# DakeQQ/Voice-Activity-Detection-VAD-ONNX

Hardware: AMD Instinct MI355X
Metric: audio frames/sec/GPU (16 kHz, 512-sample hop); RTF at batch=1 (higher is better)
Workload: dtype f32; 1 GPU; Silero-VAD f32, batch=4096 synthetic 10 s @16 kHz clips per GPU (STFT conv + conv1d stack + LSTM cell HIP, seeded synthetic weights); clips_per_gpu=4096, samples_per_clip=160000, frames_per_clip=313, parallelism=clip-sharded x1, no collective

## Files before the change

voice-activity-detection-vad-onnx_amd/csrc/silero.hip:

```cpp
#include "silero_common.h"
#include "split_scheme.h"

#include <math.h>
#include <stddef.h>
#include <stdlib.h>
#include <string.h>

namespace vadx {
namespace silero {

constexpr int ENCODER_DEFAULT = 2;

constexpr int V_LD = 100, A1_LD = 68, A2_LD = 36, A3_LD = 20, A4_LD = 20;
constexpr int V_SCR = 129 * V_LD;
constexpr int R0_FLOATS = V_SCR + 256;
constexpr int A2_OFF = 128 * A1_LD;
constexpr int A3_OFF = 0, A4_OFF = 64 * A3_LD;
constexpr int ENC_LDS_FLOATS = R0_FLOATS;
static_assert(16 * X_LDM <= R0_FLOATS && A2_OFF + 64 * A2_LD <= R0_FLOATS && 3 * ENC_LDS_FLOATS * 4 <= 160 * 1024, "encoder LDS map");

__device__ constexpr float WINO_BT[6][4] = {{0.f, -5.f, 0.f, 1.f}, {-4.f, -4.f, 1.f, 1.f}, {4.f, -4.f, -1.f, 1.f},
                                            {-2.f, -1.f, 2.f, 1.f}, {2.f, -1.f, -2.f, 1.f}, {4.f, 0.f, -5.f, 0.f}};
constexpr int ENC_THREADS = 512;

// ... 362 lines not shown
    }
    __syncthreads();

    {
        const f32x4 a4 = gemm_chain<0, 4, 4, 4>(A3, A3_LD, P + OFF_C4 + wave * 4 * FRAG + lane * 4, lane, [](int) { return 0; });
        const float bias = P[OFF_B4 + wave * 16 + i];
        f32x4 v;
#pragma unroll
        for (int r = 0; r < 4; ++r) v[r] = fmaxf(a4[r] + bias, 0.f);
        *reinterpret_cast<f32x4 *>(&A4[(wave * 16 + i) * A4_LD + 4 * q]) = v;
    }
    __syncthreads();

    {
        f32x4 acc[4][1];
#pragma unroll
        for (int g = 0; g < 4; ++g)
            acc[g][0] = *reinterpret_cast<const f32x4 *>(P + OFF_BG + g * 128 + wave * 16 + 4 * q);
        {
            const float *wl = P + OFF_IH + wave * 8 * FRAG + lane * 4;
            const float *ap = A4 + (4 * q) * A4_LD + i;
            f32x4 wcur[4], wnxt[4];
#pragma unroll
            for (int g = 0; g < 4; ++g) wcur[g] = *reinterpret_cast<const f32x4 *>(wl + g * 64 * FRAG);
#pragma unroll
            for (int S = 0; S < 8; ++S) {
                const int Sn = (S + 1 < 8) ? S + 1 : S;
#pragma unroll
                for (int g = 0; g < 4; ++g) wnxt[g] = *reinterpret_cast<const f32x4 *>(wl + g * 64 * FRAG + Sn * FRAG);
                __builtin_amdgcn_sched_barrier(0);
                const float *aps = ap + 16 * S * A4_LD;
#pragma unroll
                for (int j = 0; j < 4; ++j) {
                    const float av = aps[j * A4_LD];
#pragma unroll
                    for (int g = 0; g < 4; ++g) acc[g][0] = mfma16(wcur[g][j], av, acc[g][0]);
                }
#pragma unroll
                for (int g = 0; g < 4; ++g) wcur[g] = wnxt[g];
            }
        }
        float *dst = gx + ((size_t)t * Gws + g0 + grp) * GX_TILE_FLOATS + (size_t)wave * 4 * 256 + lane * 4;
#pragma unroll
        for (int g = 0; g < 4; ++g)
            *reinterpret_cast<f32x4 *>(dst + g * 256) = acc[g][0];
    }
}

constexpr int HS_LD = 136;
constexpr int LSTM_LDS_FLOATS = 2 * 16 * HS_LD + 2 * 8 * 16;
constexpr int LSTM_THREADS = 512;

__global__ __launch_bounds__(LSTM_THREADS, 2) void silero_lstm_kernel(
    const float *__restrict__ P, const float *__restrict__ gx, const float *__restrict__ state0,
    int B, int G, int T, float *__restrict__ probs, long long probs_stride,
    float *__restrict__ state_n) {
    extern __shared__ __attribute__((aligned(16))) float lds[];
    float *Hs = lds;
    float *part = lds + 2 * 16 * HS_LD;

    const int tid = threadIdx.x, lane = tid & 63, wave = tid >> 6;
    const int q = lane >> 4, n = lane & 15;
    const int grp = blockIdx.x;
    const long long b = (long long)grp * 16 + n;
    const bool bvalid = b < B;
    const int u0 = wave * 16 + 4 * q;

    float a[4][32];
#pragma unroll
    for (int g = 0; g < 4; ++g) {
        const float *row = P + OFF_HH + (g * 128 + wave * 16 + n) * 128 + 4 * q;
#pragma unroll
        for (int S = 0; S < 8; ++S) {
            const f32x4 w4 = *reinterpret_cast<const f32x4 *>(row + 16 * S);
            a[g][4 * S + 0] = w4[0]; a[g][4 * S + 1] = w4[1]; a[g][4 * S + 2] = w4[2]; a[g][4 * S + 3] = w4[3];
        }
    }
    f32x4 dw = *reinterpret_cast<const f32x4 *>(P + OFF_DW + u0);
    const float db = P[OFF_DB];

    f32x4 c = {0.f, 0.f, 0.f, 0.f}, h = {0.f, 0.f, 0.f, 0.f};
    if (state0 != nullptr && bvalid) {
        h = *reinterpret_cast<const f32x4 *>(state0 + b * 128 + u0);
        c = *reinterpret_cast<const f32x4 *>(state0 + ((long long)B + b) * 128 + u0);
    }
    *reinterpret_cast<f32x4 *>(&Hs[n * HS_LD + u0]) = h;
    __syncthreads();

    const float *gsrc = gx + (size_t)grp * GX_TILE_FLOATS + (size_t)wave * 4 * 256 + lane * 4;
    const size_t gstep = (size_t)G * GX_TILE_FLOATS;
    f32x4 gcur[4], gnxt[4];
#pragma unroll
    for (int g = 0; g < 4; ++g) gcur[g] = *reinterpret_cast<const f32x4 *>(gsrc + g * 256);

    int cur = 0;
    for (int t = 0; t < T; ++t) {
        const int tn = (t + 1 < T) ? t + 1 : t;
#pragma unroll
        for (int g = 0; g < 4; ++g) gnxt[g] = *reinterpret_cast<const f32x4 *>(gsrc + tn * gstep + g * 256);

        const float *hb = Hs + cur * 16 * HS_LD + n * HS_LD + 4 * q;
        f32x4 hv[8];
#pragma unroll
        for (int S = 0; S < 8; ++S) hv[S] = *reinterpret_cast<const f32x4 *>(hb + 16 * S);
        auto gate = [&](int g) {
            f32x4 acc = gcur[g];
#pragma unroll
            for (int S = 0; S < 8; ++S)
#pragma unroll
                for (int j = 0; j < 4; ++j) acc = mfma16(a[g][4 * S + j], hv[S][j], acc);
            return acc;
        };
        const f32x4 ai = gate(0), af = gate(1);
        f32x4 ig, fg, gg;
#pragma unroll
        for (int r = 0; r < 4; ++r) ig[r] = gate_sigmoid(ai[r]);
        const f32x4 ag = gate(2);
#pragma unroll
        for (int r = 0; r < 4; ++r) fg[r] = gate_sigmoid(af[r]);
        const f32x4 ao = gate(3);
        float dpart = 0.f;
#pragma unroll
        for (int r = 0; r < 4; ++r) {
            gg[r] = gate_tanh(ag[r]);
            c[r] = fg[r] * c[r] + ig[r] * gg[r];
        }
#pragma unroll
        for (int r = 0; r < 4; ++r) {
            h[r] = gate_sigmoid(ao[r]) * gate_tanh(c[r]);
            dpart = fmaf(dw[r], fmaxf(h[r], 0.f), dpart);
        }
        const int nxt = cur ^ 1;
        *reinterpret_cast<f32x4 *>(&Hs[nxt * 16 * HS_LD + n * HS_LD + u0]) = h;
        dpart += __shfl_xor(dpart, 16);
        dpart += __shfl_xor(dpart, 32);
        if (q == 0) part[(nxt * 8 + wave) * 16 + n] = dpart;
        __syncthreads();
        if (wave == 0 && lane < 16 && bvalid) {
            float s = db;
#pragma unroll
            for (int w = 0; w < 8; ++w) s += part[(nxt * 8 + w) * 16 + lane];
            probs[b * probs_stride + t] = sigmoidf_(s);
        }
        cur = nxt;
#pragma unroll
        for (int g = 0; g < 4; ++g) gcur[g] = gnxt[g];
    }
    if (state_n != nullptr && bvalid) {
        *reinterpret_cast<f32x4 *>(state_n + b * 128 + u0) = h;
        *reinterpret_cast<f32x4 *>(state_n + ((long long)B + b) * 128 + u0) = c;
    }
}

constexpr int SEG_CLIPS = 16;
__global__ void silero_segments_kernel(const float *__restrict__ probs, int B, int T,
                                       const long long *__restrict__ n_samples,
                                       vadx_silero_seg_params prm, long long *__restrict__ segs,
                                       int *__restrict__ counts, int cap) {
    const int b = blockIdx.x * blockDim.x + threadIdx.x;
    if (b >= B) return;
    const double sr = (double)prm.sampling_rate;
    const long long W = (prm.sampling_rate == 16000) ? 512 : 256;
    const double thr = prm.threshold;
    const double neg = (prm.neg_threshold < 0.0) ? fmax(thr - 0.15, 0.01) : prm.neg_threshold;
    const double min_speech = sr * prm.min_speech_duration_ms / 1000.0;
    const double pad = sr * prm.speech_pad_ms / 1000.0;
    const double max_speech = sr * prm.max_speech_duration_s - (double)W - 2.0 * pad;
    const double min_sil = sr * prm.min_silence_duration_ms / 1000.0;
    const double min_sil_at_max = sr * prm.min_silence_at_max_speech / 1000.0;
    const long long L = n_samples[b];
    const int nwin = (int)((L + W - 1) / W) < T ? (int)((L + W - 1) / W) : T;

    long long *out = segs + (size_t)b * cap * 2;
    int ns = 0;
    auto push = [&](long long s, long long e) {
        if (ns < cap) { out[2 * ns] = s; out[2 * ns + 1] = e; }
        ++ns;
    };

    auto win_floor = [&](double x) { const double q = floor(x / (double)W); return q >= 2147483647.0 ? 2147483647 : (q <= -2147483648.0 ? (int)-2147483647 - 1 : (int)q); };
    auto win_ceil = [&](double x) { const double q = ceil(x / (double)W); return q >= 2147483647.0 ? 2147483647 : (q <= -2147483648.0 ? (int)-2147483647 - 1 : (int)q); };
    auto f32_not_below = [](double x) { float f = (float)x; if ((double)f < x) f = nextafterf(f, INFINITY); return f; };
    const float thr_f = f32_not_below(thr), neg_f = f32_not_below(neg);
    const int d_sil_at_max = win_floor(min_sil_at_max), d_max_speech = win_floor(max_speech), d_min_sil = win_ceil(min_sil),
              d_min_speech = win_floor(min_speech);
    auto pushw = [&](int s_, int e_) { push((long long)s_ * W, (long long)e_ * W); };

    bool triggered = false, have_cur = false, have_possible = false;
    int cur_start = 0, temp_end = 0, prev_end = 0, next_start = 0;
    int best_end = 0, best_dur = 0;
    auto step = [&](int pos, float p) {
        if (p >= thr_f && temp_end) {
            const int gap = pos - temp_end;
            if (gap > d_sil_at_max) {
                if (!have_possible || gap > best_dur) { best_end = temp_end; best_dur = gap; }
                have_possible = true;
            }
            temp_end = 0;
            if (next_start < prev_end) next_start = pos;
        }
        if (p >= thr_f && !triggered) {
            triggered = true; cur_start = pos; have_cur = true;
            return;
        }
        if (triggered && (pos - cur_start) > d_max_speech) {
            if (prm.use_max_poss_sil_at_max_speech && have_possible) {
                prev_end = best_end;
                pushw(cur_start, prev_end);
                have_cur = false;
                next_start = prev_end + best_dur;
                if (next_start < prev_end + pos) { cur_start = next_start; have_cur = true; }
                else triggered = false;
                prev_end = next_start = temp_end = 0;
                have_possible = false;
            } else if (prev_end) {
                pushw(cur_start, prev_end);
                have_cur = false;
                if (next_start < prev_end) triggered = false;
                else { cur_start = next_start; have_cur = true; }
                prev_end = next_start = temp_end = 0;
                have_possible = false;
            } else {
                pushw(cur_start, pos);
                have_cur = false;
                prev_end = next_start = temp_end = 0;
                triggered = false;
                have_possible = false;
                return;
            }
        }
        if (p < neg_f && triggered) {
            if (!temp_end) temp_end = pos;
            const int sil_now = pos - temp_end;
            if (!prm.use_max_poss_sil_at_max_speech && sil_now > d_sil_at_max) prev_end = temp_end;
            if (sil_now < d_min_sil) return;
            if ((temp_end - cur_start) > d_min_speech) pushw(cur_start, temp_end);
            have_cur = false;
            prev_end = next_start = temp_end = 0;
            triggered = false;
            have_possible = false;
            return;
        }
        };
    const float *pr = probs + (size_t)b * T;
    for (int k0 = 0; k0 < nwin; k0 += 8) {
        float buf[8];
#pragma unroll
        for (int j = 0; j < 8; ++j) buf[j] = pr[k0 + j < T ? k0 + j : T - 1];
#pragma unroll
        for (int j = 0; j < 8; ++j)
            if (k0 + j < nwin) step(k0 + j, buf[j]);
    }
    if (have_cur && (double)(L - (long long)cur_start * W) > min_speech) push((long long)cur_start * W, L);

    const int m = ns < cap ? ns : cap;
    for (int s = 0; s < m; ++s) {
        if (s == 0) out[0] = (long long)fmax(0.0, (double)out[0] - pad);
        if (s != m - 1) {
            const long long gap = out[2 * (s + 1)] - out[2 * s + 1];
            if ((double)gap < 2.0 * pad) {
                const long long half = gap >= 0 ? gap / 2 : -((-gap + 1) / 2);
                out[2 * s + 1] += half;
                const long long ns0 = out[2 * (s + 1)] - half;
                out[2 * (s + 1)] = ns0 > 0 ? ns0 : 0;
            } else {
                out[2 * s + 1] = (long long)fmin((double)L, (double)out[2 * s + 1] + pad);
                out[2 * (s + 1)] = (long long)fmax(0.0, (double)out[2 * (s + 1)] - pad);
            }
        } else {
            out[2 * s + 1] = (long long)fmin((double)L, (double)out[2 * s + 1] + pad);
        }
    }
    counts[b] = ns;
}


}
}

using namespace vadx::silero;
using vadx::FRAG;

#define VADX_SILERO_ARITH(cfg, who)                                                                               \
    const int arith = vadx::arith_internal((cfg) ? (cfg)->arithmetic : VADX_ARITH_AUTO, ENCODER_DEFAULT);         \
    VADX_REQUIRE(arith >= 0, who ": cfg->arithmetic=%d is not one of VADX_ARITH_*", (cfg) ? (cfg)->arithmetic : 0)
static_assert(sizeof(vadx_silero_cfg) == 16 && offsetof(vadx_silero_cfg, ext) == 4 && sizeof(((vadx_silero_cfg *)nullptr)->ext) == 12,
              "vadx_silero_cfg layout");
static int rate_of(const vadx_silero_cfg *cfg) {
    const int r = cfg ? cfg->ext.sample_rate : 0;
    return (r == 0 || r == 16000) ? 16000 : (r == 8000 ? 8000 : -1);
}
#define VADX_SILERO_RATE(cfg, who)                                                                                \
    const int rate = rate_of(cfg);                                                                                \
    VADX_REQUIRE(rate > 0, who ": cfg->ext.sample_rate=%d is not 16000 or 8000 (0 = 16000)", (cfg) ? (cfg)->ext.sample_rate : 0); \
    const long long win = rate == 8000 ? 256 : 512, ctx = win / 8

extern "C" int vadx_silero_range_flag(const float *packed, int reset, uint32_t *flag_host, float *amax_host, void *stream) {
    VADX_REQUIRE(packed && flag_host, "vadx_silero_range_flag: NULL argument");
    return vadx::range_flag_read(packed + OFF_HFLAG + 1, reset, flag_host, amax_host, stream);
}

extern "C" size_t vadx_silero_workspace_bytes(int batch, int steps) {
    if (batch <= 0 || steps <= 0) return 0;
    const size_t G = ((size_t)batch + 15) / 16;
    return G * (size_t)steps * GX_TILE_FLOATS * sizeof(float);
}

template <typename S>
int vadx::silero::silero_encode_launch(const float *packed, const S *src, float in_scale, long long n_valid, long long row_stride,
                                       long long origin, int batch, int steps, void *ws, size_t ws_bytes, void *stream,
                                       const vadx_silero_cfg *cfg, int first_group, int total_batch) {
    VADX_SILERO_ARITH(cfg, "silero");
    VADX_SILERO_RATE(cfg, "silero");
    (void)ctx;
    VADX_REQUIRE(packed && src && ws, "silero: NULL pointer argument");
    VADX_REQUIRE(batch > 0 && steps > 0, "silero: batch=%d steps=%d must be positive", batch, steps);
    VADX_REQUIRE((reinterpret_cast<uintptr_t>(packed) & 15) == 0 && (reinterpret_cast<uintptr_t>(ws) & 15) == 0,
                 "silero: packed weights and workspace must be 16-byte aligned");
    if (total_batch <= 0) total_batch = batch;
    const int Gws = (total_batch + 15) / 16;
    const int G = (batch + 15) / 16;
    VADX_REQUIRE(first_group >= 0 && first_group + G <= Gws, "silero: clip groups [%d, %d) outside the workspace's %d", first_group,
                 first_group + G, Gws);
    if (ws_bytes < vadx_silero_workspace_bytes(total_batch, steps)) {
        vadx::set_error("silero: workspace %zu B < required %zu B", ws_bytes, vadx_silero_workspace_bytes(total_batch, steps));
        return VADX_ENOSPACE;
    }
    const long long nblk = (long long)G * steps;
    VADX_REQUIRE(nblk < (1LL << 31), "silero: too many tiles (%lld)", nblk);
    if (win == 256)
        return silero8k_encode_launch<S>(arith, packed, src, in_scale, n_valid, row_stride, origin, batch, G, steps, Gws, first_group,
                                         static_cast<float *>(ws), stream);
    if (arith == 2)
        return silero_encode_h2_launch<S>(packed, src, in_scale, n_valid, row_stride, origin, batch, G, steps, Gws, first_group,
                                          static_cast<float *>(ws), stream);
    if (arith == 1)
        return silero_encode_split_launch<S>(packed, src, in_scale, n_valid, row_stride, origin, batch, G, steps, Gws, first_group,
                                             static_cast<float *>(ws), stream);
    VADX_DYN_LDS(silero_encode_kernel<S>, ENC_LDS_FLOATS * sizeof(float));
    hipLaunchKernelGGL(silero_encode_kernel<S>, dim3((unsigned)nblk), dim3(ENC_THREADS), ENC_LDS_FLOATS * sizeof(float),
                       static_cast<hipStream_t>(stream), packed, src, in_scale, n_valid, row_stride, origin, batch, G, steps,
                       Gws, first_group, static_cast<float *>(ws));
    VADX_HIP_TRY(hipGetLastError());
    return VADX_OK;
}

int vadx::silero::silero_recur_launch(const float *packed, const void *ws, size_t ws_bytes, int batch, int steps,
                                      const float *state0, float *probs, long long probs_stride, float *state_n, void *stream,
                                      const vadx_silero_cfg *cfg) {
    VADX_SILERO_ARITH(cfg, "silero");
    VADX_SILERO_RATE(cfg, "silero");
    (void)win; (void)ctx;
    VADX_REQUIRE(packed && ws && probs, "silero: NULL pointer argument");
    VADX_REQUIRE(batch > 0 && steps > 0, "silero: batch=%d steps=%d must be positive", batch, steps);
    if (ws_bytes < vadx_silero_workspace_bytes(batch, steps)) {
        vadx::set_error("silero: workspace %zu B < required %zu B", ws_bytes, vadx_silero_workspace_bytes(batch, steps));
        return VADX_ENOSPACE;
    }
    const int G = (batch + 15) / 16;
    if (arith == 2)
        return silero_lstm_h2_launch(packed, static_cast<const float *>(ws), state0, batch, G, steps, probs, probs_stride, state_n, stream);
    if (arith == 1)
        return silero_lstm_split_launch(packed, static_cast<const float *>(ws), state0, batch, G, steps, probs, probs_stride, state_n, stream);
    hipLaunchKernelGGL(silero_lstm_kernel, dim3(G), dim3(LSTM_THREADS), LSTM_LDS_FLOATS * sizeof(float),
                       static_cast<hipStream_t>(stream), packed, static_cast<const float *>(ws), state0, batch, G, steps,
                       probs, probs_stride, state_n);
    VADX_HIP_TRY(hipGetLastError());
    return VADX_OK;
}

template int vadx::silero::silero_encode_launch<float>(const float *, const float *, float, long long, long long, long long, int, int,
                                                       void *, size_t, void *, const vadx_silero_cfg *, int, int);
template int vadx::silero::silero_encode_launch<int16_t>(const float *, const int16_t *, float, long long, long long, long long, int, int,
                                                         void *, size_t, void *, const vadx_silero_cfg *, int, int);

static int silero_run(const float *packed, const float *src, long long n_valid, long long row_stride,
                      long long origin, int batch, int steps, const float *state0, float *probs,
                      long long probs_stride, float *state_n, void *ws, size_t ws_bytes, void *stream, const vadx_silero_cfg *cfg) {
    int rc = silero_encode_launch(packed, src, 1.0f, n_valid, row_stride, origin, batch, steps, ws, ws_bytes, stream, cfg);
    if (rc != VADX_OK) return rc;
    return silero_recur_launch(packed, ws, ws_bytes, batch, steps, state0, probs, probs_stride, state_n, stream, cfg);
}

extern "C" int vadx_silero_encode(const float *packed, const float *audio, int batch, int64_t n_samples,
                                  int64_t row_stride, void *workspace, size_t workspace_bytes, void *stream, const vadx_silero_cfg *cfg) {
    VADX_SILERO_RATE(cfg, "vadx_silero_encode");
    VADX_REQUIRE(n_samples > 0 && row_stride >= n_samples, "vadx_silero_encode: n_samples=%lld row_stride=%lld",
                 (long long)n_samples, (long long)row_stride);
    const long long steps = (n_samples + win - 1) / win;
    VADX_REQUIRE(steps < (1LL << 30), "vadx_silero_encode: clip too long");
    return silero_encode_launch(packed, audio, 1.0f, n_samples, row_stride, -ctx, batch, (int)steps, workspace, workspace_bytes, stream, cfg);
}

extern "C" int vadx_silero_encode_pcm16(const float *packed, const int16_t *audio, float scale, int batch, int64_t n_samples,
                                        int64_t row_stride, void *workspace, size_t workspace_bytes, void *stream, const vadx_silero_cfg *cfg) {
    VADX_SILERO_RATE(cfg, "vadx_silero_encode_pcm16");
    VADX_REQUIRE(n_samples > 0 && row_stride >= n_samples, "vadx_silero_encode_pcm16: n_samples=%lld row_stride=%lld",
                 (long long)n_samples, (long long)row_stride);
    const long long steps = (n_samples + win - 1) / win;
    VADX_REQUIRE(steps < (1LL << 30), "vadx_silero_encode_pcm16: clip too long");
    return silero_encode_launch(packed, audio, scale, n_samples, row_stride, -ctx, batch, (int)steps, workspace, workspace_bytes, stream, cfg);
}

extern "C" int vadx_silero_encode_pcm16_part(const float *packed, const int16_t *audio, float scale, int batch, int64_t n_samples,
                                             int64_t row_stride, int first_clip, int total_batch, void *workspace,
                                             size_t workspace_bytes, void *stream, const vadx_silero_cfg *cfg) {
    VADX_SILERO_RATE(cfg, "vadx_silero_encode_pcm16_part");
    VADX_REQUIRE(n_samples > 0 && row_stride >= n_samples, "vadx_silero_encode_pcm16_part: n_samples=%lld row_stride=%lld",
                 (long long)n_samples, (long long)row_stride);
    VADX_REQUIRE(first_clip >= 0 && first_clip % 16 == 0 && first_clip + batch <= total_batch,
                 "vadx_silero_encode_pcm16_part: first_clip=%d must be a multiple of 16 and first_clip + batch <= total_batch=%d",
                 first_clip, total_batch);
    const long long steps = (n_samples + win - 1) / win;
    VADX_REQUIRE(steps < (1LL << 30), "vadx_silero_encode_pcm16_part: clip too long");
    return silero_encode_launch(packed, audio, scale, n_samples, row_stride, -ctx, batch, (int)steps, workspace, workspace_bytes, stream,
                                cfg, first_clip / 16, total_batch);
}

extern "C" int vadx_silero_recur(const float *packed, const void *workspace, size_t workspace_bytes, int batch,
                                 int steps, const float *state0, float *probs, float *state_n, void *stream, const vadx_silero_cfg *cfg) {
    return silero_recur_launch(packed, workspace, workspace_bytes, batch, steps, state0, probs, steps, state_n, stream, cfg);
}

extern "C" int vadx_silero_encode_span(const float *packed, const float *audio, int batch, int64_t n_samples,
                                       int64_t row_stride, int first_step, int n_steps, void *workspace,
                                       size_t workspace_bytes, void *stream, const vadx_silero_cfg *cfg) {
    VADX_SILERO_RATE(cfg, "vadx_silero_encode_span");
    VADX_REQUIRE(n_samples > 0 && row_stride >= n_samples, "vadx_silero_encode_span: n_samples=%lld row_stride=%lld",
                 (long long)n_samples, (long long)row_stride);
    const long long steps = (n_samples + win - 1) / win;
    VADX_REQUIRE(first_step >= 0 && n_steps > 0 && (long long)first_step + n_steps <= steps,
                 "vadx_silero_encode_span: span [%d, %d + %d) outside the clip's %lld windows", first_step, first_step, n_steps, steps);
    return silero_encode_launch(packed, audio, 1.0f, n_samples, row_stride, (long long)first_step * win - ctx, batch, n_steps,
                                workspace, workspace_bytes, stream, cfg);
}

extern "C" int vadx_silero_recur_span(const float *packed, const void *workspace, size_t workspace_bytes, int batch,
                                      int n_steps, const float *state0, float *probs, int64_t probs_stride,
                                      float *state_n, void *stream, const vadx_silero_cfg *cfg) {
    VADX_REQUIRE(probs_stride >= n_steps, "vadx_silero_recur_span: probs_stride=%lld < n_steps=%d", (long long)probs_stride, n_steps);
    return silero_recur_launch(packed, workspace, workspace_bytes, batch, n_steps, state0, probs, probs_stride, state_n, stream, cfg);
}

extern "C" int vadx_silero_step(const float *packed, const float *input, const float *state, int64_t sr,
                                int batch, float *out, float *state_n, void *workspace,
                                size_t workspace_bytes, void *stream, const vadx_silero_cfg *cfg) {
    VADX_SILERO_RATE(cfg, "vadx_silero_step");
    VADX_REQUIRE(sr == rate, "Supported sampling rates: [%d] (got %lld; vadx_silero_cfg.ext.sample_rate selects the network)", rate, (long long)sr);
    VADX_REQUIRE(state && state_n, "vadx_silero_step: state / state_n must not be NULL");
    return silero_run(packed, input, win + ctx, win + ctx, 0, batch, 1, state, out, 1, state_n, workspace, workspace_bytes, stream, cfg);
}

extern "C" int vadx_silero_clips(const float *packed, const float *audio, int batch, int64_t n_samples,
                                 int64_t row_stride, float *probs, float *state_n, void *workspace,
                                 size_t workspace_bytes, void *stream, const vadx_silero_cfg *cfg) {
    VADX_SILERO_RATE(cfg, "vadx_silero_clips");
    VADX_REQUIRE(n_samples > 0 && row_stride >= n_samples, "vadx_silero_clips: n_samples=%lld row_stride=%lld",
                 (long long)n_samples, (long long)row_stride);
    const long long steps = (n_samples + win - 1) / win;
    VADX_REQUIRE(steps < (1LL << 30), "vadx_silero_clips: clip too long");
    return silero_run(packed, audio, n_samples, row_stride, -ctx, batch, (int)steps, nullptr, probs, steps,
                      state_n, workspace, workspace_bytes, stream, cfg);
}

extern "C" int vadx_silero_segments(const float *probs, int batch, int steps, const int64_t *n_samples,
                                    const vadx_silero_seg_params *params, int64_t *segments,
                                    int32_t *counts, int cap, void *stream) {
    VADX_REQUIRE(probs && n_samples && params && segments && counts, "vadx_silero_segments: NULL pointer argument");
    VADX_REQUIRE(batch > 0 && steps > 0 && cap > 0, "vadx_silero_segments: batch/steps/cap must be positive");
    VADX_REQUIRE(params->sampling_rate == 16000 || params->sampling_rate == 8000,
                 "Currently silero VAD models support 8000 and 16000 (or multiply of 16000) sample rates");
    hipLaunchKernelGGL(silero_segments_kernel, dim3((batch + SEG_CLIPS - 1) / SEG_CLIPS), dim3(SEG_CLIPS), 0, static_cast<hipStream_t>(stream),
                       probs, batch, steps, reinterpret_cast<const long long *>(n_samples), *params,
                       reinterpret_cast<long long *>(segments), counts, cap);
    VADX_HIP_TRY(hipGetLastError());
    return VADX_OK;
}
```

voice-activity-detection-vad-onnx_amd/csrc/silero_h2.hip:

```cpp
#include "silero_common.h"
#include "split2.h"

#define H2_IDS()                                                                                           \
    int t_ = tid0;                                                                                         \
    asm volatile("" : "+v"(t_));                                                                           \
    const int tid = t_, lane = tid & 63, wave = tid >> 6, q = lane >> 4, i = lane & 15;                    \
    (void)tid; (void)lane; (void)wave; (void)q; (void)i

namespace vadx {
namespace silero {

constexpr int H2_THREADS = 512;
constexpr int H2_WAVES_PER_SIMD = 4;
constexpr int H2_AHS = 2, H2_AH1 = 2;
constexpr int H2_EO_PL = 8192, H2_EO_KG = 1024;
constexpr int H2_PL128 = 16384, H2_FR128 = 4096;
constexpr int H2_SCR = 32768;
constexpr int H2_EXC2 = 36864, H2_EXC3 = 45056;
constexpr int H2_C2 = 53248, H2_PL2 = 4096, H2_FR2 = 2048;
constexpr int H2_R1 = 65536, H2_T3 = 4096, H2_PL3 = 2048;
constexpr int H2_C4 = 0, H2_T4 = 8192, H2_PL4 = 4096;
constexpr int H2_NSUB = 4;
constexpr int H2_LDS_BYTES = H2_R1 + H2_NSUB * H2_T3;
static_assert(16 * X_LDM * 4 <= H2_EXC3 && H2_EXC3 + 4096 <= H2_C2 && H2_C2 + 2 * H2_PL2 <= H2_R1, "fp16 x 2 encoder LDS map: a tile");
// ... 356 lines not shown
            }
        }
        f32x4 s2[2] = {join2(hi[0], mid[0]), join2(hi[1], mid[1])};
        float *exc = reinterpret_cast<float *>(smem + H2_EXC2);
        if (kh == 1) {
#pragma unroll
            for (int o = 0; o < 2; ++o) *reinterpret_cast<f32x4 *>(exc + ((rt * 2 + o) * 64 + lane) * 4) = s2[o];
        }
        __syncthreads();
        if (kh == 0) {
            const f32x4 bias = ldg4(P + OFF_B2 + 16 * rt + 4 * q);
#pragma unroll
            for (int o = 0; o < 2; ++o) {
                const f32x4 other = *reinterpret_cast<const f32x4 *>(exc + ((rt * 2 + o) * 64 + lane) * 4);
                f32x4 y;
#pragma unroll
                for (int r = 0; r < 4; ++r) y[r] = fmaxf(s2[o][r] + other[r] + bias[r], 0.f);
                store_h4(smem + H2_C2 + o * H2_FR2, H2_PL2, 4 * rt + q, i, y, amax);
            }
        }
    }
    f16x8 pre_3[2][2];
    {
        H2_IDS();
        const float *w3 = P + OFF_H3 + ((wave & 3) * 2 + (wave >> 2)) * (2 * 2 * HF);
        load_a2(pre_3[0], w3, lane);
        load_a2(pre_3[1], w3 + 2 * HF, lane);
    }
    __syncthreads();

    {
        H2_IDS();
        const int rt = wave & 3, th = wave >> 2;
        f32x4 hi = {0.f, 0.f, 0.f, 0.f}, mid = hi;
#pragma unroll
        for (int kc = 0; kc < 2; ++kc) {
            f16x8 b[2];
            load_b2(b, smem + H2_C2 + th * H2_FR2, H2_PL2, kc, q, i);
            mfma_split3(pre_3[kc], b, hi, mid);
        }
        float *exc = reinterpret_cast<float *>(smem + H2_EXC3);
        if (th == 1) *reinterpret_cast<f32x4 *>(exc + (rt * 64 + lane) * 4) = join2(hi, mid);
        __syncthreads();
        if (th == 0) {
            const f32x4 bias = ldg4(P + OFF_B3 + 16 * rt + 4 * q);
            const f32x4 s3 = join2(hi, mid), other = *reinterpret_cast<const f32x4 *>(exc + (rt * 64 + lane) * 4);
            f32x4 y;
#pragma unroll
            for (int r = 0; r < 4; ++r) y[r] = fmaxf(s3[r] + other[r] + bias[r], 0.f);
            store_h4(smem + H2_R1 + sub * H2_T3, H2_PL3, 4 * rt + q, i, y, amax);
        }
    }
    }

    auto ih_s = [](int j) { return 4 * ((j >> 1) & 3) + 2 * (j >> 3) + (j & 1); };
    __syncthreads();
    {
        H2_IDS();
        const int rt = wave;
        const f32x4 bias = ldg4(P + OFF_B4 + 16 * rt + 4 * q);
        f32x4 hi[NSUB], mid[NSUB];
#pragma unroll
        for (int sb = 0; sb < NSUB; ++sb) { hi[sb] = bias; mid[sb] = f32x4{0.f, 0.f, 0.f, 0.f}; }
        const float *w4 = P + OFF_H4 + wave * (2 * 2 * HF);
        f16x8 a[2][2];
        load_a2(a[0], w4, lane);
        load_a2(a[1], w4 + 2 * HF, lane);
#pragma unroll
        for (int kc = 0; kc < 2; ++kc)
#pragma unroll
            for (int sb = 0; sb < NSUB; ++sb) {
                if (sb < nvalid) {
                    f16x8 b[2];
                    load_b2(b, smem + H2_R1 + sb * H2_T3, H2_PL3, kc, q, i);
                    mfma_split3(a[kc], b, hi[sb], mid[sb]);
                }
            }
#pragma unroll
        for (int sb = 0; sb < NSUB; ++sb) {
            if (sb < nvalid) {
                const f32x4 s = join2(hi[sb], mid[sb]);
                f32x4 y;
#pragma unroll
                for (int r = 0; r < 4; ++r) y[r] = fmaxf(s[r], 0.f);
                store_h4(smem + H2_C4 + sb * H2_T4, H2_PL4, 4 * rt + q, i, y, amax);
            }
        }
        const bool bad = !(amax <= H_MAX);
        if (__ballot(bad) != 0ULL && lane == 0) reinterpret_cast<unsigned *>(scr)[128 + wave] = 1u;
        else if (lane == 0) reinterpret_cast<unsigned *>(scr)[128 + wave] = 0u;
    }
    __syncthreads();

    {
        H2_IDS();
        const unsigned *bw = reinterpret_cast<const unsigned *>(scr) + 128;
        const bool poison = __builtin_amdgcn_readfirstlane((int)(bw[0] | bw[1] | bw[2] | bw[3] | bw[4] | bw[5] | bw[6] | bw[7])) != 0;
        const float *wq = P + OFF_HIH + wave * (4 * 4 * 2 * HF);
        f16x8 a[2][2][2];
#pragma unroll
        for (int gg = 0; gg < 2; ++gg) load_a2(a[0][gg], wq + ih_s(gg) * 2 * HF, lane);
#pragma unroll
        for (int gh = 0; gh < 2; ++gh) {
            f32x4 hi[NSUB][2], mid[NSUB][2];
#pragma unroll
            for (int gg = 0; gg < 2; ++gg) {
                const f32x4 bg = ldg4(P + OFF_BG + (2 * gh + gg) * 128 + wave * 16 + 4 * q);
#pragma unroll
                for (int sb = 0; sb < NSUB; ++sb) { hi[sb][gg] = bg; mid[sb][gg] = f32x4{0.f, 0.f, 0.f, 0.f}; }
            }
#pragma unroll
            for (int kc = 0; kc < 4; ++kc) {
                const int j = 8 * gh + 2 * kc;
#pragma unroll
                for (int gg = 0; gg < 2; ++gg)
                    if (j + 2 < 16) load_a2(a[((j >> 1) + 1) & 1][gg], wq + ih_s(j + 2 + gg) * 2 * HF, lane);
                const f16x8 (&ac)[2][2] = a[(j >> 1) & 1];
#pragma unroll
                for (int sb = 0; sb < NSUB; ++sb) {
                    if (sb < nvalid) {
                        f16x8 b[2];
                        load_b2(b, smem + H2_C4 + sb * H2_T4, H2_PL4, kc, q, i);
#pragma unroll
                        for (int gg = 0; gg < 2; ++gg)
                            mfma_split3(ac[gg], b, hi[sb][gg], mid[sb][gg]);
                    }
                }
            }
#pragma unroll
            for (int sb = 0; sb < NSUB; ++sb) {
                if (sb >= nvalid) continue;
                const int t_s = (int)(blk / G) * NSUB + sb, grp_s = (int)(blk % G);
                float *dst = gx + ((size_t)t_s * Gws + g0 + grp_s) * GX_TILE_FLOATS + (size_t)wave * 4 * 256 + lane * 4;
                if (!poison) {
#pragma unroll
                    for (int gg = 0; gg < 2; ++gg) *reinterpret_cast<f32x4 *>(dst + (2 * gh + gg) * 256) = join2(hi[sb][gg], mid[sb][gg]);
                } else {
                    const float qnan = __builtin_nanf("");
#pragma unroll
                    for (int gg = 0; gg < 2; ++gg) *reinterpret_cast<f32x4 *>(dst + (2 * gh + gg) * 256) = f32x4{qnan, qnan, qnan, qnan};
                }
            }
        }
    }
    }
    if (!(amax <= H_MAX)) {
        unsigned *fl = reinterpret_cast<unsigned *>(const_cast<float *>(P)) + OFF_HFLAG + 1;
        atomicOr(fl, 1u);
        atomicMax(fl + 1, __float_as_uint(amax));
    }
}

constexpr int LH_HPL = 4096, LH_HBUF = 8192;
constexpr int LH_PART = 2 * LH_HBUF;
constexpr int LH_BYTES = LH_PART + 1024;
constexpr int LH_GX_AHEAD = 3;

__global__ __launch_bounds__(512, 2) void silero_lstm_h2_kernel(
    const float *__restrict__ P, const float *__restrict__ gx, const float *__restrict__ state0,
    int B, int G, int T, float *__restrict__ probs, long long probs_stride, float *__restrict__ state_n) {
    extern __shared__ __attribute__((aligned(16))) unsigned char smem[];
    float *part = reinterpret_cast<float *>(smem + LH_PART);

    const int tid = threadIdx.x, lane = tid & 63, wave = tid >> 6;
    const int q = lane >> 4, n = lane & 15;
    const int grp = blockIdx.x;
    const long long b = (long long)grp * 16 + n;
    const bool bvalid = b < B;
    const int u0 = wave * 16 + 4 * q;
    if (ldg1(P + OFF_HFLAG) == 0.f) {
        if (tid == 0 && grp == 0) atomicOr(reinterpret_cast<unsigned *>(const_cast<float *>(P)) + OFF_HFLAG + 1, 2u);
        if (wave == 0 && lane < 16 && bvalid)
            for (int t = 0; t < T; ++t) probs[b * probs_stride + t] = __builtin_nanf("");
        return;
    }

    f16x8 a[4][4][2];
    {
        const float *wq = P + OFF_HHH + (size_t)wave * (4 * 4 * 2 * HF);
#pragma unroll
        for (int g = 0; g < 4; ++g)
#pragma unroll
            for (int kc = 0; kc < 4; ++kc) load_a2(a[g][kc], wq + (g * 4 + kc) * 2 * HF, lane);
    }
    const f32x4 dwh = ldg4(P + OFF_DW + u0) * 0.5f;
    const float db = P[OFF_DB];

    float amax = 0.f;
    f32x4 c = {0.f, 0.f, 0.f, 0.f}, h = {0.f, 0.f, 0.f, 0.f};
    if (state0 != nullptr && bvalid) {
        h = *reinterpret_cast<const f32x4 *>(state0 + b * 128 + u0);
        c = *reinterpret_cast<const f32x4 *>(state0 + ((long long)B + b) * 128 + u0);
    }
    store_h4(smem, LH_HPL, 4 * wave + q, n, h, amax);
    __syncthreads();

    const float *gsrc = gx + (size_t)grp * GX_TILE_FLOATS + (size_t)wave * 4 * 256 + lane * 4;
    const size_t gstep = (size_t)G * GX_TILE_FLOATS;
    constexpr int GA = LH_GX_AHEAD;
    f32x4 gq[GA][4];
#pragma unroll
    for (int j = 0; j < GA; ++j) {
        const int tj = j < T ? j : T - 1;
#pragma unroll
        for (int g = 0; g < 4; ++g) gq[j][g] = *reinterpret_cast<const f32x4 *>(gsrc + tj * gstep + g * 256);
    }

    int cur = 0;
    for (int t0 = 0; t0 < T; t0 += GA) {
#pragma unroll
    for (int j = 0; j < GA; ++j) {
        const int t = t0 + j;
        if (t >= T) break;
        f32x4 hi[4], mid[4];
#pragma unroll
        for (int g = 0; g < 4; ++g) { hi[g] = gq[j][g]; mid[g] = f32x4{0.f, 0.f, 0.f, 0.f}; }
        {
            const int tn = (t + GA < T) ? t + GA : T - 1;
#pragma unroll
            for (int g = 0; g < 4; ++g) gq[j][g] = *reinterpret_cast<const f32x4 *>(gsrc + tn * gstep + g * 256);
        }
        const unsigned char *hb = smem + cur * LH_HBUF;
        float dpart = 0.f;
#pragma unroll
        for (int kc = 0; kc < 4; ++kc) {
            f16x8 bb[2];
            load_b2(bb, hb, LH_HPL, kc, q, n);
#pragma unroll
            for (int g = 0; g < 4; ++g) mid[g] = mfma_f16(a[g][kc][1], bb[0], mid[g]);
#pragma unroll
            for (int g = 0; g < 4; ++g) mid[g] = mfma_f16(a[g][kc][0], bb[1], mid[g]);
#pragma unroll
            for (int g = 0; g < 4; ++g) hi[g] = mfma_f16(a[g][kc][0], bb[0], hi[g]);
        }
#pragma unroll
        for (int r = 0; r < 4; ++r) {
            const float ig = gate_sigmoid(fmaf(mid[0][r], H1_INV, hi[0][r])), fg = gate_sigmoid(fmaf(mid[1][r], H1_INV, hi[1][r]));
            const float gg = gate_tanh(fmaf(mid[2][r], H1_INV, hi[2][r])), og = gate_sigmoid(fmaf(mid[3][r], H1_INV, hi[3][r]));
            c[r] = fg * c[r] + ig * gg;
            h[r] = og * gate_tanh(c[r]);
            dpart = fmaf(dwh[r], h[r] + __builtin_fabsf(h[r]), dpart);
        }
        const int nxt = cur ^ 1;
        store_h4(smem + nxt * LH_HBUF, LH_HPL, 4 * wave + q, n, h, amax);
        dpart += __shfl_xor(dpart, 16);
        dpart += __shfl_xor(dpart, 32);
        if (q == 0) part[(nxt * 8 + wave) * 16 + n] = dpart;
        __syncthreads();
        if (wave == 0 && lane < 16 && bvalid) {
            float s = db;
#pragma unroll
            for (int w = 0; w < 8; ++w) s += part[(nxt * 8 + w) * 16 + lane];
            probs[b * probs_stride + t] = sigmoidf_(s);
        }
        cur = nxt;
    }
    }
    if (state_n != nullptr && bvalid) {
        *reinterpret_cast<f32x4 *>(state_n + b * 128 + u0) = h;
        *reinterpret_cast<f32x4 *>(state_n + ((long long)B + b) * 128 + u0) = c;
    }
    if (!(amax <= H_MAX)) {
        unsigned *fl = reinterpret_cast<unsigned *>(const_cast<float *>(P)) + OFF_HFLAG + 1;
        atomicOr(fl, 1u);
        atomicMax(fl + 1, __float_as_uint(amax));
    }
    __syncthreads();
    if (__ballot(!(amax <= H_MAX)) != 0ULL && lane == 0) reinterpret_cast<unsigned *>(part)[wave] = 1u;
    else if (lane == 0) reinterpret_cast<unsigned *>(part)[wave] = 0u;
    __syncthreads();
    {
        const unsigned *bw = reinterpret_cast<const unsigned *>(part);
        if ((bw[0] | bw[1] | bw[2] | bw[3] | bw[4] | bw[5] | bw[6] | bw[7]) != 0u && wave == 0 && lane < 16 && bvalid)
            for (int t = 0; t < T; ++t) probs[b * probs_stride + t] = __builtin_nanf("");
    }
}

int silero_lstm_h2_launch(const float *packed, const float *gx, const float *state0, int batch, int G, int steps, float *probs,
                          long long probs_stride, float *state_n, void *stream) {
    hipLaunchKernelGGL(silero_lstm_h2_kernel, dim3(G), dim3(512), LH_BYTES, static_cast<hipStream_t>(stream), packed, gx, state0, batch, G,
                       steps, probs, probs_stride, state_n);
    VADX_HIP_TRY(hipGetLastError());
    return VADX_OK;
}

template <typename S>
int silero_encode_h2_launch(const float *packed, const S *src, float in_scale, long long n_valid, long long row_stride,
                            long long origin, int batch, int G, int steps, int Gws, int first_group, float *gx, void *stream) {
    constexpr int NS = H2_NSUB;
    constexpr int LDS = H2_LDS_BYTES;
    VADX_DYN_LDS((silero_encode_h2_kernel<S, NS>), LDS);
    const long long nblk = (long long)G * ((steps + NS - 1) / NS);
    hipLaunchKernelGGL((silero_encode_h2_kernel<S, NS>), dim3((unsigned)nblk), dim3(H2_THREADS), LDS, static_cast<hipStream_t>(stream),
                       packed, src, in_scale, n_valid, row_stride, origin, batch, G, steps, Gws, first_group, gx);
    VADX_HIP_TRY(hipGetLastError());
    return VADX_OK;
}
template int silero_encode_h2_launch<float>(const float *, const float *, float, long long, long long, long long, int, int, int, int, int, float *, void *);
template int silero_encode_h2_launch<int16_t>(const float *, const int16_t *, float, long long, long long, long long, int, int, int, int, int, float *, void *);

}
}
```

Baseline: 318.0 million frames/s.

## Wave-parallel segment scan with ballots and batch LSTM probability stores per block

The segments kernel now gives each clip a whole wavefront. It loads 64 probabilities at once, builds threshold bitmasks with ballots and jumps to the next event with ctz, instead of stepping through every frame serially on a single thread. Separately, the h2 LSTM kernel keeps per-step partial dot products in a 32-slot ring in LDS and writes sigmoid probabilities in bursts every 16 steps from 256 threads. Before, 16 lanes wrote one probability each step, which gave scattered stores on the serial recurrence path. The cost is more LDS per block, extra branching logic, and a thread fence at the end.

```diff
diff --git a/voice-activity-detection-vad-onnx_amd/csrc/silero.hip b/voice-activity-detection-vad-onnx_amd/csrc/silero.hip
--- a/voice-activity-detection-vad-onnx_amd/csrc/silero.hip
+++ b/voice-activity-detection-vad-onnx_amd/csrc/silero.hip
@@ -538,12 +538,13 @@
     }
 }
 
-constexpr int SEG_CLIPS = 16;
-__global__ void silero_segments_kernel(const float *__restrict__ probs, int B, int T,
+constexpr int SEG_WAVES = 4;
+__global__ __launch_bounds__(64 * SEG_WAVES) void silero_segments_kernel(const float *__restrict__ probs, int B, int T,
                                        const long long *__restrict__ n_samples,
                                        vadx_silero_seg_params prm, long long *__restrict__ segs,
                                        int *__restrict__ counts, int cap) {
-    const int b = blockIdx.x * blockDim.x + threadIdx.x;
+    const int lane = threadIdx.x & 63;
+    const int b = blockIdx.x * SEG_WAVES + __builtin_amdgcn_readfirstlane((int)(threadIdx.x >> 6));
     if (b >= B) return;
     const double sr = (double)prm.sampling_rate;
     const long long W = (prm.sampling_rate == 16000) ? 512 : 256;
@@ -560,7 +561,7 @@
     long long *out = segs + (size_t)b * cap * 2;
     int ns = 0;
     auto push = [&](long long s, long long e) {
-        if (ns < cap) { out[2 * ns] = s; out[2 * ns + 1] = e; }
+        if (ns < cap && lane == 0) { out[2 * ns] = s; out[2 * ns + 1] = e; }
         ++ns;
     };
 
@@ -568,77 +569,92 @@
     auto win_ceil = [&](double x) { const double q = ceil(x / (double)W); return q >= 2147483647.0 ? 2147483647 : (q <= -2147483648.0 ? (int)-2147483647 - 1 : (int)q); };
     auto f32_not_below = [](double x) { float f = (float)x; if ((double)f < x) f = nextafterf(f, INFINITY); return f; };
     const float thr_f = f32_not_below(thr), neg_f = f32_not_below(neg);
-    const int d_sil_at_max = win_floor(min_sil_at_max), d_max_speech = win_floor(max_speech), d_min_sil = win_ceil(min_sil),
-              d_min_speech = win_floor(min_speech);
+    const int d_sil_at_max = __builtin_amdgcn_readfirstlane(win_floor(min_sil_at_max)), d_max_speech = __builtin_amdgcn_readfirstlane(win_floor(max_speech)),
+              d_min_sil = __builtin_amdgcn_readfirstlane(win_ceil(min_sil)), d_min_speech = __builtin_amdgcn_readfirstlane(win_floor(min_speech));
     auto pushw = [&](int s_, int e_) { push((long long)s_ * W, (long long)e_ * W); };
 
     bool triggered = false, have_cur = false, have_possible = false;
     int cur_start = 0, temp_end = 0, prev_end = 0, next_start = 0;
     int best_end = 0, best_dur = 0;
-    auto step = [&](int pos, float p) {
-        if (p >= thr_f && temp_end) {
-            const int gap = pos - temp_end;
-            if (gap > d_sil_at_max) {
-                if (!have_possible || gap > best_dur) { best_end = temp_end; best_dur = gap; }
-                have_possible = true;
-            }
-            temp_end = 0;
-            if (next_start < prev_end) next_start = pos;
-        }
-        if (p >= thr_f && !triggered) {
-            triggered = true; cur_start = pos; have_cur = true;
-            return;
-        }
-        if (triggered && (pos - cur_start) > d_max_speech) {
-            if (prm.use_max_poss_sil_at_max_speech && have_possible) {
-                prev_end = best_end;
-                pushw(cur_start, prev_end);
-                have_cur = false;
-                next_start = prev_end + best_dur;
-                if (next_start < prev_end + pos) { cur_start = next_start; have_cur = true; }
-                else triggered = false;
-                prev_end = next_start = temp_end = 0;
-                have_possible = false;
-            } else if (prev_end) {
-                pushw(cur_start, prev_end);
-                have_cur = false;
-                if (next_start < prev_end) triggered = false;
-                else { cur_start = next_start; have_cur = true; }
-                prev_end = next_start = temp_end = 0;
-                have_possible = false;
-            } else {
-                pushw(cur_start, pos);
+    const float *pr = probs + (size_t)b * T;
+    const float qnan = __builtin_nanf("");
+    float p = lane < nwin ? pr[lane] : qnan;
+    for (int k0 = 0; k0 < nwin; k0 += 64) {
+        const float pn = (nwin - k0 > 64 + lane) ? pr[k0 + 64 + lane] : qnan;
+        const unsigned long long ge_m = __ballot(p >= thr_f), lt_m = __ballot(p < neg_f);
+        const int len = nwin - k0 < 64 ? nwin - k0 : 64;
+        int i = 0;
+        while (i < len) {
+            const unsigned long long m = (triggered ? (lt_m | (temp_end ? ge_m : 0ULL)) : ge_m) & (~0ULL << i);
+            int nx = m ? (int)__builtin_ctzll(m) : 64;
+            if (triggered) {
+                int last;
+                const bool nowhere = __builtin_sadd_overflow(cur_start, d_max_speech, &last) || last == 2147483647;
+                const int li = (nowhere || last + 1 >= k0 + len) ? 64 : (last + 1 <= k0 + i ? i : last + 1 - k0);
+                nx = li < nx ? li : nx;
+            }
+            if (nx >= len) break;
+            const int pos = k0 + nx;
+            const bool ge = (ge_m >> nx) & 1ULL, lt = (lt_m >> nx) & 1ULL;
+            i = nx + 1;
+            if (ge && temp_end) {
+                const int gap = pos - temp_end;
+                if (gap > d_sil_at_max) {
+                    if (!have_possible || gap > best_dur) { best_end = temp_end; best_dur = gap; }
+                    have_possible = true;
+                }
+                temp_end = 0;
+                if (next_start < prev_end) next_start = pos;
+            }
+            if (ge && !triggered) {
+                triggered = true; cur_start = pos; have_cur = true;
+                continue;
+            }
+            if (triggered && (pos - cur_start) > d_max_speech) {
+                if (prm.use_max_poss_sil_at_max_speech && have_possible) {
+                    prev_end = best_end;
+                    pushw(cur_start, prev_end);
+                    have_cur = false;
+                    next_start = prev_end + best_dur;
+                    if (next_start < prev_end + pos) { cur_start = next_start; have_cur = true; }
+                    else triggered = false;
+                    prev_end = next_start = temp_end = 0;
+                    have_possible = false;
+                } else if (prev_end) {
+                    pushw(cur_start, prev_end);
+                    have_cur = false;
+                    if (next_start < prev_end) triggered = false;
+                    else { cur_start = next_start; have_cur = true; }
+                    prev_end = next_start = temp_end = 0;
+                    have_possible = false;
+                } else {
+                    pushw(cur_start, pos);
+                    have_cur = false;
+                    prev_end = next_start = temp_end = 0;
+                    triggered = false;
+                    have_possible = false;
+                    continue;
+                }
+            }
+            if (lt && triggered) {
+                if (!temp_end) temp_end = pos;
+                const int sil_now = pos - temp_end;
+                if (!prm.use_max_poss_sil_at_max_speech && sil_now > d_sil_at_max) prev_end = temp_end;
+                if (sil_now < d_min_sil) continue;
+                if ((temp_end - cur_start) > d_min_speech) pushw(cur_start, temp_end);
                 have_cur = false;
                 prev_end = next_start = temp_end = 0;
                 triggered = false;
                 have_possible = false;
-                return;
-            }
-        }
-        if (p < neg_f && triggered) {
-            if (!temp_end) temp_end = pos;
-            const int sil_now = pos - temp_end;
-            if (!prm.use_max_poss_sil_at_max_speech && sil_now > d_sil_at_max) prev_end = temp_end;
-            if (sil_now < d_min_sil) return;
-            if ((temp_end - cur_start) > d_min_speech) pushw(cur_start, temp_end);
-            have_cur = false;
-            prev_end = next_start = temp_end = 0;
-            triggered = false;
-            have_possible = false;
-            return;
-        }
-        };
-    const float *pr = probs + (size_t)b * T;
-    for (int k0 = 0; k0 < nwin; k0 += 8) {
-        float buf[8];
-#pragma unroll
-        for (int j = 0; j < 8; ++j) buf[j] = pr[k0 + j < T ? k0 + j : T - 1];
-#pragma unroll
-        for (int j = 0; j < 8; ++j)
-            if (k0 + j < nwin) step(k0 + j, buf[j]);
+                continue;
+            }
+        }
+        if (nwin - k0 <= 64) break;
+        p = pn;
     }
     if (have_cur && (double)(L - (long long)cur_start * W) > min_speech) push((long long)cur_start * W, L);
 
+    if (lane != 0) return;
     const int m = ns < cap ? ns : cap;
     for (int s = 0; s < m; ++s) {
         if (s == 0) out[0] = (long long)fmax(0.0, (double)out[0] - pad);
@@ -856,7 +872,7 @@
     VADX_REQUIRE(batch > 0 && steps > 0 && cap > 0, "vadx_silero_segments: batch/steps/cap must be positive");
     VADX_REQUIRE(params->sampling_rate == 16000 || params->sampling_rate == 8000,
                  "Currently silero VAD models support 8000 and 16000 (or multiply of 16000) sample rates");
-    hipLaunchKernelGGL(silero_segments_kernel, dim3((batch + SEG_CLIPS - 1) / SEG_CLIPS), dim3(SEG_CLIPS), 0, static_cast<hipStream_t>(stream),
+    hipLaunchKernelGGL(silero_segments_kernel, dim3((batch + SEG_WAVES - 1) / SEG_WAVES), dim3(64 * SEG_WAVES), 0, static_cast<hipStream_t>(stream),
                        probs, batch, steps, reinterpret_cast<const long long *>(n_samples), *params,
                        reinterpret_cast<long long *>(segments), counts, cap);
     VADX_HIP_TRY(hipGetLastError());
diff --git a/voice-activity-detection-vad-onnx_amd/csrc/silero_h2.hip b/voice-activity-detection-vad-onnx_amd/csrc/silero_h2.hip
--- a/voice-activity-detection-vad-onnx_amd/csrc/silero_h2.hip
+++ b/voice-activity-detection-vad-onnx_amd/csrc/silero_h2.hip
@@ -532,8 +532,10 @@
 }
 
 constexpr int LH_HPL = 4096, LH_HBUF = 8192;
+constexpr int LH_BLK = 16;
+constexpr int LH_SLOT = 8 * 16 + 4;
 constexpr int LH_PART = 2 * LH_HBUF;
-constexpr int LH_BYTES = LH_PART + 1024;
+constexpr int LH_BYTES = LH_PART + 2 * LH_BLK * LH_SLOT * 4;
 constexpr int LH_GX_AHEAD = 3;
 
 __global__ __launch_bounds__(512, 2) void silero_lstm_h2_kernel(
@@ -625,13 +627,18 @@
         store_h4(smem + nxt * LH_HBUF, LH_HPL, 4 * wave + q, n, h, amax);
         dpart += __shfl_xor(dpart, 16);
         dpart += __shfl_xor(dpart, 32);
-        if (q == 0) part[(nxt * 8 + wave) * 16 + n] = dpart;
+        if (q == 0) part[(t & (2 * LH_BLK - 1)) * LH_SLOT + wave * 16 + n] = dpart;
         __syncthreads();
-        if (wave == 0 && lane < 16 && bvalid) {
-            float s = db;
-#pragma unroll
-            for (int w = 0; w < 8; ++w) s += part[(nxt * 8 + w) * 16 + lane];
-            probs[b * probs_stride + t] = sigmoidf_(s);
+        if ((t & (LH_BLK - 1)) == LH_BLK - 1 || t == T - 1) {
+            const int fc = tid >> 4, fs = tid & (LH_BLK - 1), t_blk = t & ~(LH_BLK - 1);
+            const long long fb = (long long)grp * 16 + fc;
+            if (tid < 16 * LH_BLK && fb < B && t_blk + fs <= t) {
+                const float *pp = part + ((t_blk + fs) & (2 * LH_BLK - 1)) * LH_SLOT + fc;
+                float s = db;
+#pragma unroll
+                for (int w = 0; w < 8; ++w) s += pp[w * 16];
+                probs[fb * probs_stride + t_blk + fs] = sigmoidf_(s);
+            }
         }
         cur = nxt;
     }
@@ -645,6 +652,7 @@
         atomicOr(fl, 1u);
         atomicMax(fl + 1, __float_as_uint(amax));
     }
+    __threadfence();
     __syncthreads();
     if (__ballot(!(amax <= H_MAX)) != 0ULL && lane == 0) reinterpret_cast<unsigned *>(part)[wave] = 1u;
     else if (lane == 0) reinterpret_cast<unsigned *>(part)[wave] = 0u;
```

Result: faster. 325.1 million frames/s (median of 6 runs) (+2.2%).
